# basilevh/occlusions-4d

Hardware: AMD Instinct MI355X
Metric: 4D query-points/sec (encode+decode) at n_points=14336 (higher is better)
Workload: dtype f32; 1 GPU; GREATER inference (BASELINE configs[1]): n_points=14336 video_len=12 num_sample=524288 (-> 534528 grid queries) implicit_batch_size=32768 (decoded in mini-batches of 32256 = 3584 workgroups of 9 queries; every query is decoded, results do not depend on the split), seeded random-init weights; abstract_points=531, outputs_per_query=5, parallelism=single GPU, schedule=sequential, rccl_ranks=1, decode_streams=2, decode_chunk=32256

## Files before the change

### occlusions-4d_amd/csrc/tile.hpp

```cpp
#pragma once
#include "common.hpp"

namespace {

typedef float f32x2 __attribute__((ext_vector_type(2)));
typedef float f32x4 __attribute__((ext_vector_type(4)));
typedef float f32x16 __attribute__((ext_vector_type(16)));
typedef unsigned u32x2 __attribute__((ext_vector_type(2)));
typedef unsigned u32x4 __attribute__((ext_vector_type(4)));

template <typename T>
__device__ __forceinline__ unsigned lds_addr(const T* p) {
  return (unsigned)(uintptr_t)(const __attribute__((address_space(3))) T*)p;
}

template <typename T>
__device__ __forceinline__ void dma_frag(const T* __restrict__ src_frag, unsigned lds_dst, unsigned lane16) {
  unsigned keep;
  asm volatile("s_mov_b32 %0, m0\n\ts_mov_b32 m0, %2\n\ts_nop 0\n\tglobal_load_lds_dwordx4 %1, %3\n\ts_mov_b32 m0, %0"
               : "=&s"(keep) : "v"(lane16), "s"(lds_dst), "s"(src_frag) : "memory");
}
__device__ __forceinline__ void dma_wait() { asm volatile("s_waitcnt vmcnt(0)" ::: "memory"); }

__device__ __forceinline__ f32x4 relu4(f32x4 v) {
  v.x = fmaxf(v.x, 0.f); v.y = fmaxf(v.y, 0.f); v.z = fmaxf(v.z, 0.f); v.w = fmaxf(v.w, 0.f);
  return v;
}

struct Pair { float lo, hi; };
__device__ __forceinline__ Pair swap16(float x, float y) {
  const auto r = __builtin_amdgcn_permlane16_swap(__float_as_uint(x), __float_as_uint(y), false, false);
  return Pair{__uint_as_float(r[0]), __uint_as_float(r[1])};
}
__device__ __forceinline__ Pair swap32(float x, float y) {
  const auto r = __builtin_amdgcn_permlane32_swap(__float_as_uint(x), __float_as_uint(y), false, false);
  return Pair{__uint_as_float(r[0]), __uint_as_float(r[1])};
}

__device__ __forceinline__ void mfma16x2(const f32x4 a0, const f32x4 a1, const f32x4 b0, const f32x4 b1, f32x4& c0, f32x4& c1) {
  c0 = __builtin_amdgcn_mfma_f32_16x16x4f32(a0.x, b0.x, c0, 0, 0, 0);
  c1 = __builtin_amdgcn_mfma_f32_16x16x4f32(a1.x, b1.x, c1, 0, 0, 0);
  c0 = __builtin_amdgcn_mfma_f32_16x16x4f32(a0.y, b0.y, c0, 0, 0, 0);
  c1 = __builtin_amdgcn_mfma_f32_16x16x4f32(a1.y, b1.y, c1, 0, 0, 0);
  c0 = __builtin_amdgcn_mfma_f32_16x16x4f32(a0.z, b0.z, c0, 0, 0, 0);
  c1 = __builtin_amdgcn_mfma_f32_16x16x4f32(a1.z, b1.z, c1, 0, 0, 0);
  c0 = __builtin_amdgcn_mfma_f32_16x16x4f32(a0.w, b0.w, c0, 0, 0, 0);
  c1 = __builtin_amdgcn_mfma_f32_16x16x4f32(a1.w, b1.w, c1, 0, 0, 0);
}
__device__ __forceinline__ void mfma16x2_a(const f32x4 a, const f32x4 b0, const f32x4 b1, f32x4& c0, f32x4& c1) {
  mfma16x2(a, a, b0, b1, c0, c1);
}
__device__ __forceinline__ void mfma16x2_b(const f32x4 a0, const f32x4 a1, const f32x4 b, f32x4& c0, f32x4& c1) {
  mfma16x2(a0, a1, b, b, c0, c1);
}

}
```

### occlusions-4d_amd/csrc/trunk.hip

```cpp
#include "tile.hpp"

namespace {

constexpr int TH = 416;
constexpr int TKG = TH / 16;
constexpr int TNS = TH / 32;
constexpr int FRAG_FLOATS = 256;
constexpr int STAGE_FRAGS = 2 * TKG;
constexpr int STAGE_FLOATS = STAGE_FRAGS * FRAG_FLOATS;
constexpr int TROWS = 128;

struct TrunkArgs {
  const float* x; int64_t ldx;
  float* y; int64_t ldy;
  const float* w0p; const float* b0;
  const float* w1p; const float* b1;
  const float* res; int64_t ldr;
  const float* zconst; const float* ztab; int64_t ldz; const int32_t* zidx; const float* zw; int kz;
  int n;
  int n_stages;
  int relu_in;
  const float* mask; int64_t ldm;
};

__device__ __forceinline__ void dma_stage(const float* __restrict__ src, const float* dst, int wave, int lane) {
#pragma unroll
  for (int i = 0; i < 7; ++i) {
    const int c = wave + 8 * i;
    if (c < STAGE_FRAGS) dma_frag(src + c * FRAG_FLOATS, lds_addr(dst) + (unsigned)c * (FRAG_FLOATS * 4), (unsigned)lane * 16u);
  }
}

__device__ __forceinline__ void dma_part(const float* __restrict__ src, const float* dst, int wave, int lane, int i) {
  const int c = wave + 8 * i;
  if (c < STAGE_FRAGS) dma_frag(src + c * FRAG_FLOATS, lds_addr(dst) + (unsigned)c * (FRAG_FLOATS * 4), (unsigned)lane * 16u);
}

__device__ __forceinline__ void interp_into(const TrunkArgs& a, int rowc, int g, f32x4* out) {
#pragma unroll
  for (int t = 0; t < TKG; ++t) {
    const f32x4 c = *reinterpret_cast<const f32x4*>(a.zconst + 16 * t + 4 * g);
    out[t].x += c.x; out[t].y += c.y; out[t].z += c.z; out[t].w += c.w;
  }
  for (int j = 0; j < a.kz; ++j) {
    const float w = a.zw[(int64_t)rowc * a.kz + j];
    const float* zr = a.ztab + (int64_t)a.zidx[(int64_t)rowc * a.kz + j] * a.ldz + 4 * g;
#pragma unroll
    for (int t = 0; t < TKG; ++t) {
      const f32x4 z = *reinterpret_cast<const f32x4*>(zr + 16 * t);
      out[t].x = fmaf(w, z.x, out[t].x); out[t].y = fmaf(w, z.y, out[t].y);
      out[t].z = fmaf(w, z.z, out[t].z); out[t].w = fmaf(w, z.w, out[t].w);
    }
  }
}

__global__ __launch_bounds__(512, 2) void resblock_kernel(const TrunkArgs a) {
  __shared__ __attribute__((aligned(16))) float bufA[STAGE_FLOATS];
  __shared__ __attribute__((aligned(16))) float bufB[STAGE_FLOATS];
  __shared__ __attribute__((aligned(16))) float s_b0[TH];
  const int tid = threadIdx.x, lane = tid & 63, wave = __builtin_amdgcn_readfirstlane(tid >> 6);
  const int r = lane & 15, g = lane >> 4;
  const int row = blockIdx.x * TROWS + wave * 16 + r;
  const int rowc = min(row, a.n - 1);

  dma_stage(a.w0p, bufA, wave, lane);
  if (tid < TH) s_b0[tid] = a.b0[tid];
  f32x4 xr[TKG], yacc[TKG];
  {
    const float* xp = a.x + (int64_t)rowc * a.ldx + 4 * g;
#pragma unroll
    for (int t = 0; t < TKG; ++t) {
#ifdef OCC4D_TR_NOPRO
      const f32x4 v = {(float)t, (float)g, (float)r, 1.f};
#else
      const f32x4 v = *reinterpret_cast<const f32x4*>(xp + 16 * t);
#endif
      const f32x4 b = *reinterpret_cast<const f32x4*>(a.b1 + 16 * t + 4 * g);
      xr[t] = relu4(v);
      yacc[t].x = v.x + b.x; yacc[t].y = v.y + b.y; yacc[t].z = v.z + b.z; yacc[t].w = v.w + b.w;
    }
  }
  dma_wait();
  __syncthreads();
  const float* const fa = bufA + lane * 4;
  const float* const fb = bufB + lane * 4;

#ifdef OCC4D_TR_STAMP
  unsigned long long tacc[4] = {0, 0, 0, 0};
  unsigned long long tprev = __builtin_amdgcn_s_memtime();
  const unsigned long long tstart = tprev;
#define STAMP(i) { const unsigned long long tn = __builtin_amdgcn_s_memtime(); tacc[i] += tn - tprev; tprev = tn; }
#else
#define STAMP(i)
#endif
  asm volatile("; OCC4D_MARK loop");
#pragma clang loop unroll(disable)
  for (int j = 0; j < TNS; ++j) {
    f32x4 h0 = *reinterpret_cast<const f32x4*>(s_b0 + 32 * j + 4 * g);
    f32x4 h1 = *reinterpret_cast<const f32x4*>(s_b0 + 32 * j + 16 + 4 * g);
    {
      f32x4 wa = *reinterpret_cast<const f32x4*>(fa);
      f32x4 wb = *reinterpret_cast<const f32x4*>(fa + TKG * FRAG_FLOATS);
#pragma unroll
      for (int t = 0; t < TKG; ++t) {
#ifndef OCC4D_TR_NODMA
        if (t >= 2 && t <= 20 && (t - 2) % 3 == 0) dma_part(a.w1p + (int64_t)j * STAGE_FLOATS, bufB, wave, lane, (t - 2) / 3);
#endif
        const f32x4 ca = wa, cb = wb;
        if (t + 1 < TKG) {
          wa = *reinterpret_cast<const f32x4*>(fa + (t + 1) * FRAG_FLOATS);
          wb = *reinterpret_cast<const f32x4*>(fa + (TKG + t + 1) * FRAG_FLOATS);
        }
        __builtin_amdgcn_sched_barrier(0);
        mfma16x2_b(ca, cb, xr[t], h0, h1);
        __builtin_amdgcn_sched_barrier(0);
      }
    }
    h0 = relu4(h0);
    h1 = relu4(h1);
    STAMP(0)
#ifndef OCC4D_TR_NOBAR
    dma_wait();
    __syncthreads();
#endif
    STAMP(1)
    {
      f32x4 wa = *reinterpret_cast<const f32x4*>(fb);
      f32x4 wb = *reinterpret_cast<const f32x4*>(fb + 2 * FRAG_FLOATS);
#pragma unroll
      for (int q = 0; q < TKG; ++q) {
        const int p = q >> 1, tt = q & 1;
#ifndef OCC4D_TR_NODMA
        if (q >= 2 && q <= 20 && (q - 2) % 3 == 0) dma_part(a.w0p + (int64_t)(j + 1) * STAGE_FLOATS, bufA, wave, lane, (q - 2) / 3);
#endif
        const f32x4 ca = wa, cb = wb;
        if (q + 1 < TKG) {
          const int pn = (q + 1) >> 1, tn = (q + 1) & 1;
          wa = *reinterpret_cast<const f32x4*>(fb + (4 * pn + tn) * FRAG_FLOATS);
          wb = *reinterpret_cast<const f32x4*>(fb + (4 * pn + 2 + tn) * FRAG_FLOATS);
        }
        __builtin_amdgcn_sched_barrier(0);
        mfma16x2_b(ca, cb, tt ? h1 : h0, yacc[2 * p], yacc[2 * p + 1]);
        __builtin_amdgcn_sched_barrier(0);
      }
    }
    STAMP(2)
#ifndef OCC4D_TR_NOBAR
    dma_wait();
    __syncthreads();
#endif
    STAMP(3)
  }
  asm volatile("; OCC4D_MARK epilogue");
#ifdef OCC4D_TR_STAMP
  if (lane == 0 && a.zw) {
    unsigned long long* o = (unsigned long long*)a.zw + (size_t)(blockIdx.x * 8 + wave) * 6;
    o[0] = tacc[0]; o[1] = tacc[1]; o[2] = tacc[2]; o[3] = tacc[3]; o[4] = tprev - tstart; o[5] = tstart;
  }
#endif
  if (a.ztab) interp_into(a, rowc, g, yacc);
#ifdef OCC4D_TR_NOEPI
  {
    float tsum = 0.f;
#pragma unroll
    for (int t = 0; t < TKG; ++t) tsum += yacc[t].x + yacc[t].y + yacc[t].z + yacc[t].w;
    if (tsum == 123.456f) a.y[0] = tsum;
    return;
  }
#endif
  if (row < a.n) {
    float* yp = a.y + (int64_t)row * a.ldy + 4 * g;
#pragma unroll
    for (int t = 0; t < TKG; ++t) *reinterpret_cast<f32x4*>(yp + 16 * t) = yacc[t];
  }
}

__device__ __forceinline__ void rowlin_stage(const TrunkArgs& a, int s, const float* __restrict__ frag, const f32x4* xr,
                                             int row, int rowc, int g, const float* next_src, const float* next_dst,
                                             int wave, int lane) {
  const int c0 = 32 * s + 4 * g;
  const f32x4 bz0 = *reinterpret_cast<const f32x4*>(a.b0 + c0);
  const f32x4 bz1 = *reinterpret_cast<const f32x4*>(a.b0 + c0 + 16);
  f32x4 o0 = {0.f, 0.f, 0.f, 0.f}, o1 = {0.f, 0.f, 0.f, 0.f};
  f32x4 r0 = {0.f, 0.f, 0.f, 0.f}, r1 = {0.f, 0.f, 0.f, 0.f};
  if (a.res) {
    r0 = *reinterpret_cast<const f32x4*>(a.res + (int64_t)rowc * a.ldr + c0);
    r1 = *reinterpret_cast<const f32x4*>(a.res + (int64_t)rowc * a.ldr + c0 + 16);
  }
  {
    f32x4 wa = *reinterpret_cast<const f32x4*>(frag);
    f32x4 wb = *reinterpret_cast<const f32x4*>(frag + TKG * FRAG_FLOATS);
#pragma unroll
    for (int t = 0; t < TKG; ++t) {
      if (t >= 2 && t <= 20 && (t - 2) % 3 == 0) dma_part(next_src, next_dst, wave, lane, (t - 2) / 3);
      const f32x4 ca = wa, cb = wb;
      if (t + 1 < TKG) {
        wa = *reinterpret_cast<const f32x4*>(frag + (t + 1) * FRAG_FLOATS);
        wb = *reinterpret_cast<const f32x4*>(frag + (TKG + t + 1) * FRAG_FLOATS);
      }
      __builtin_amdgcn_sched_barrier(0);
      mfma16x2_b(ca, cb, xr[t], o0, o1);
      __builtin_amdgcn_sched_barrier(0);
    }
  }
  o0.x += bz0.x + r0.x; o0.y += bz0.y + r0.y; o0.z += bz0.z + r0.z; o0.w += bz0.w + r0.w;
  o1.x += bz1.x + r1.x; o1.y += bz1.y + r1.y; o1.z += bz1.z + r1.z; o1.w += bz1.w + r1.w;
  if (a.ztab) {
    const f32x4 ca = *reinterpret_cast<const f32x4*>(a.zconst + c0);
    const f32x4 cb = *reinterpret_cast<const f32x4*>(a.zconst + c0 + 16);
    o0.x += ca.x; o0.y += ca.y; o0.z += ca.z; o0.w += ca.w;
    o1.x += cb.x; o1.y += cb.y; o1.z += cb.z; o1.w += cb.w;
    for (int j = 0; j < a.kz; ++j) {
      const float w = a.zw[(int64_t)rowc * a.kz + j];
      const float* zr = a.ztab + (int64_t)a.zidx[(int64_t)rowc * a.kz + j] * a.ldz + c0;
      const f32x4 za = *reinterpret_cast<const f32x4*>(zr);
      const f32x4 zb = *reinterpret_cast<const f32x4*>(zr + 16);
      o0.x = fmaf(w, za.x, o0.x); o0.y = fmaf(w, za.y, o0.y); o0.z = fmaf(w, za.z, o0.z); o0.w = fmaf(w, za.w, o0.w);
      o1.x = fmaf(w, zb.x, o1.x); o1.y = fmaf(w, zb.y, o1.y); o1.z = fmaf(w, zb.z, o1.z); o1.w = fmaf(w, zb.w, o1.w);
    }
  }
  if (a.mask) {
    const f32x4 m0 = *reinterpret_cast<const f32x4*>(a.mask + (int64_t)rowc * a.ldm + c0);
    const f32x4 m1 = *reinterpret_cast<const f32x4*>(a.mask + (int64_t)rowc * a.ldm + c0 + 16);
    o0.x = m0.x > 0.f ? o0.x : 0.f; o0.y = m0.y > 0.f ? o0.y : 0.f; o0.z = m0.z > 0.f ? o0.z : 0.f; o0.w = m0.w > 0.f ? o0.w : 0.f;
    o1.x = m1.x > 0.f ? o1.x : 0.f; o1.y = m1.y > 0.f ? o1.y : 0.f; o1.z = m1.z > 0.f ? o1.z : 0.f; o1.w = m1.w > 0.f ? o1.w : 0.f;
  }
  if (row < a.n) {
    float* yp = a.y + (int64_t)row * a.ldy + c0;
    *reinterpret_cast<f32x4*>(yp) = o0;
    *reinterpret_cast<f32x4*>(yp + 16) = o1;
  }
}

__global__ __launch_bounds__(512, 2) void rowlin_kernel(const TrunkArgs a) {
  __shared__ __attribute__((aligned(16))) float bufA[STAGE_FLOATS];
  __shared__ __attribute__((aligned(16))) float bufB[STAGE_FLOATS];
  const int tid = threadIdx.x, lane = tid & 63, wave = __builtin_amdgcn_readfirstlane(tid >> 6);
  const int r = lane & 15, g = lane >> 4;
  const int row = blockIdx.x * TROWS + wave * 16 + r;
  const int rowc = min(row, a.n - 1);
  dma_stage(a.w0p, bufA, wave, lane);
  f32x4 xr[TKG];
  {
    const float* xp = a.x + (int64_t)rowc * a.ldx + 4 * g;
#pragma unroll
    for (int t = 0; t < TKG; ++t) {
      const f32x4 v = *reinterpret_cast<const f32x4*>(xp + 16 * t);
      xr[t] = a.relu_in ? relu4(v) : v;
    }
  }
  dma_wait();
  __syncthreads();
#pragma clang loop unroll(disable)
  for (int s = 0; s < a.n_stages; s += 2) {
    rowlin_stage(a, s, bufA + lane * 4, xr, row, rowc, g, a.w0p + (int64_t)(s + 1) * STAGE_FLOATS, bufB, wave, lane);
    dma_wait();
    __syncthreads();
    if (s + 1 < a.n_stages)
      rowlin_stage(a, s + 1, bufB + lane * 4, xr, row, rowc, g, a.w0p + (int64_t)(s + 2) * STAGE_FLOATS, bufA, wave, lane);
    dma_wait();
    __syncthreads();
  }
}

int rowlin_launch(const char* who, const float* x, int64_t ldx, float* y, int64_t ldy, const float* w_packed, const float* b,
                  int n_out, int relu_in, const float* res, int64_t ldr, const float* zconst, const float* ztab, int64_t ldz,
                  const int32_t* zidx, const float* zw, int kz, bool masked, const float* mask, int64_t ldm, int n,
                  void* stream) {
  if (n == 0) return OCC4D_OK;
  TrunkArgs a{x, ldx, y, ldy, w_packed, b, nullptr, nullptr, res, ldr, zconst, ztab, ldz, zidx, zw, kz, n,
              n_out / 32, relu_in, mask, ldm};
  if (int rc = occ4d::check_rowlin_args(a, who, TH, 32, n_out, masked)) return rc;
  rowlin_kernel<<<occ4d::cdiv(n, TROWS), 512, 0, (hipStream_t)stream>>>(a);
  return occ4d::check_launch(who);
}

}

extern "C" int occ4d_trunk_width(void) { return TH; }
extern "C" int64_t occ4d_trunk_packed_floats(int n_out) { return (int64_t)(n_out / 32 + 1) * STAGE_FLOATS; }

extern "C" int occ4d_resblock_f32(const float* x, int64_t ldx, float* y, int64_t ldy, const float* w0_packed,
                                  const float* b0, const float* w1_packed, const float* b1, const float* zconst,
                                  const float* ztab, int64_t ldz, const int32_t* zidx, const float* zw, int kz, int n,
                                  void* stream) {
  TrunkArgs a{x, ldx, y, ldy, w0_packed, b0, w1_packed, b1, nullptr, 0, zconst, ztab, ldz, zidx, zw, kz, n, TNS, 1, nullptr, 0};
  if (n == 0) return OCC4D_OK;
  if (int rc = occ4d::check_trunk_args(a, "occ4d_resblock_f32", TH)) return rc;
  OCC4D_REQUIRE(w1_packed && b1 && ((uintptr_t)w1_packed % 16) == 0 && ((uintptr_t)b1 % 16) == 0 && ldy >= TH,
                "occ4d_resblock_f32: second layer weights / bias missing or misaligned");
  resblock_kernel<<<occ4d::cdiv(n, TROWS), 512, 0, (hipStream_t)stream>>>(a);
  return occ4d::check_launch("occ4d_resblock_f32");
}

extern "C" int occ4d_rowlin_f32(const float* x, int64_t ldx, float* y, int64_t ldy, const float* w_packed,
                                const float* b, int n_out, int relu_in, const float* res, int64_t ldr,
                                const float* zconst, const float* ztab, int64_t ldz, const int32_t* zidx,
                                const float* zw, int kz, int n, void* stream) {
  return rowlin_launch("occ4d_rowlin_f32", x, ldx, y, ldy, w_packed, b, n_out, relu_in, res, ldr, zconst, ztab, ldz, zidx, zw,
                       kz, false, nullptr, 0, n, stream);
}

extern "C" int occ4d_rowlin_masked_f32(const float* x, int64_t ldx, float* y, int64_t ldy, const float* w_packed,
                                       const float* b, int n_out, int relu_in, const float* res, int64_t ldr,
                                       const float* mask, int64_t ldm, int n, void* stream) {
  return rowlin_launch("occ4d_rowlin_masked_f32", x, ldx, y, ldy, w_packed, b, n_out, relu_in, res, ldr, nullptr, nullptr, 0,
                       nullptr, nullptr, 0, true, mask, ldm, n, stream);
}
```

### profiles/ablate_trunk.py

```python
import ctypes as C
import os
import subprocess
import sys

import torch

ROOT = os.path.dirname(os.path.dirname(os.path.abspath(__file__)))
sys.path.insert(0, ROOT)
import occlusions4d_amd as pk

CSRC = os.path.join(ROOT, 'occlusions-4d_amd', 'csrc')
VARIANTS = {
    'base': [],
    'nodma': ['-DOCC4D_TR_NODMA'],
    'nobar': ['-DOCC4D_TR_NOBAR'],
    'nodma-nobar': ['-DOCC4D_TR_NODMA', '-DOCC4D_TR_NOBAR'],
    'nopro': ['-DOCC4D_TR_NOPRO'],
    'noepi': ['-DOCC4D_TR_NOEPI'],
    'nopro-noepi': ['-DOCC4D_TR_NOPRO', '-DOCC4D_TR_NOEPI'],
    'bare-loop': ['-DOCC4D_TR_NOPRO', '-DOCC4D_TR_NOEPI', '-DOCC4D_TR_NODMA', '-DOCC4D_TR_NOBAR'],
}


def main():
    n, H = 32256, 416
    x = torch.randn(n, H, device='cuda')
    w0 = torch.randn(H, H, device='cuda') * 0.05
    w1 = torch.randn(H, H, device='cuda') * 0.05
    b = torch.randn(H, device='cuda')
    y = torch.empty(n, H, device='cuda')
    p0, p1 = pk.ops.pack_trunk_rows(w0), pk.ops.pack_trunk_cols(w1)
    names = sys.argv[1:] or list(VARIANTS)
    extra = os.environ.get('OCC4D_ABLATE_EXTRA', '').split()
    for name in names:
        out = '/tmp/trunk_%s.so' % name
        subprocess.run(['hipcc', '--offload-arch=gfx950', '-O3', '-std=c++17', '-ffp-contract=off', '-fPIC', '-shared',
                        '-I' + os.path.join(ROOT, 'include'), '-I' + CSRC] + VARIANTS[name] + extra +
                       [os.path.join(CSRC, 'trunk.hip'), os.path.join(CSRC, 'error.hip'), '-o', out], check=True)
        lib = C.CDLL(out)
        fn = lib.occ4d_resblock_f32
        fn.restype = C.c_int
        fn.argtypes = pk._lib.SIGNATURES['occ4d_resblock_f32'][1]
        run = lambda: fn(x.data_ptr(), H, y.data_ptr(), H, p0.data_ptr(), b.data_ptr(), p1.data_ptr(), b.data_ptr(),
                         None, None, 0, None, None, 0, n, None)
        assert run() == 0
        torch.cuda.synchronize()
        e0, e1 = torch.cuda.Event(enable_timing=True), torch.cuda.Event(enable_timing=True)
        e0.record()
        for _ in range(20):
            run()
        e1.record()
        torch.cuda.synchronize()
        us = e0.elapsed_time(e1) / 20 * 1e3
        print('%-14s %8.1f us  %6.1f TFLOP/s  %.3f of peak' % (name, us, 4.0 * n * H * H / us / 1e6, 4.0 * n * H * H / us / 1e6 / 157.3),
              flush=True)


if __name__ == '__main__':
    main()
```

Measured before the change: 4.579 million query-points/s.

## Overlap trunk prologue loads and output stores with MFMA weight stages

The resblock and rowlin kernels now issue their input-row and bias loads as asynchronous inline-asm global loads. Each row tile is waited on with a per-tile vmcnt just before its first MFMA use, so the prologue latency overlaps the first GEMM stage. The resblock output stores are spread across the final stage's MFMA groups, and rowlin defers each stage's store into the next stage. The point is to hide global-memory latency at kernel start and end. The price is fragile hand-computed vmcnt counts that depend on the DMA schedule, plus heavy template recursion.

```diff
diff --git a/occlusions-4d_amd/csrc/tile.hpp b/occlusions-4d_amd/csrc/tile.hpp
--- a/occlusions-4d_amd/csrc/tile.hpp
+++ b/occlusions-4d_amd/csrc/tile.hpp
@@ -21,6 +21,23 @@
                : "=&s"(keep) : "v"(lane16), "s"(lds_dst), "s"(src_frag) : "memory");
 }
 __device__ __forceinline__ void dma_wait() { asm volatile("s_waitcnt vmcnt(0)" ::: "memory"); }
+
+template <int BYTE_OFF>
+__device__ __forceinline__ void load4_async(f32x4& dst, const float* base) {
+  asm volatile("global_load_dwordx4 %0, %1, off offset:%2" : "=v"(dst) : "v"(base), "n"(BYTE_OFF) : "memory");
+}
+__device__ __forceinline__ void load1_async(float& dst, const float* p) {
+  asm volatile("global_load_dword %0, %1, off" : "=v"(dst) : "v"(p) : "memory");
+}
+template <int N>
+__device__ __forceinline__ void vm_wait(f32x4& a) { asm volatile("s_waitcnt vmcnt(%1)" : "+v"(a) : "n"(N) : "memory"); }
+template <int N>
+__device__ __forceinline__ void vm_wait(f32x4& a, f32x4& b) {
+  asm volatile("s_waitcnt vmcnt(%2)" : "+v"(a), "+v"(b) : "n"(N) : "memory");
+}
+template <int N>
+__device__ __forceinline__ void vm_wait(float& a) { asm volatile("s_waitcnt vmcnt(%1)" : "+v"(a) : "n"(N) : "memory"); }
+__device__ __forceinline__ void lds_barrier() { asm volatile("s_waitcnt lgkmcnt(0)\n\ts_barrier" ::: "memory"); }
 
 __device__ __forceinline__ f32x4 relu4(f32x4 v) {
   v.x = fmaxf(v.x, 0.f); v.y = fmaxf(v.y, 0.f); v.z = fmaxf(v.z, 0.f); v.w = fmaxf(v.w, 0.f);
diff --git a/occlusions-4d_amd/csrc/trunk.hip b/occlusions-4d_amd/csrc/trunk.hip
--- a/occlusions-4d_amd/csrc/trunk.hip
+++ b/occlusions-4d_amd/csrc/trunk.hip
@@ -54,34 +54,144 @@
   }
 }
 
+constexpr int ROW_LOADS =
+#ifdef OCC4D_TR_NOPRO
+    0;
+#else
+    TKG;
+#endif
+__host__ __device__ constexpr int tile_wait_count(int t) {
+#ifdef OCC4D_TR_NODMA
+  return ROW_LOADS ? TKG - 1 - t : 0;
+#else
+  return (ROW_LOADS ? TKG - 1 - t : 0) + (t <= 2 ? 0 : ((t - 3) / 3 + 1 < 6 ? (t - 3) / 3 + 1 : 6));
+#endif
+}
+
+template <int T = 0>
+__device__ __forceinline__ void issue_row_tiles(const float* xp, f32x4* v, int g, int r) {
+  if constexpr (T < TKG) {
+#ifdef OCC4D_TR_NOPRO
+    v[T] = f32x4{(float)T, (float)g, (float)r, 1.f};
+#else
+    load4_async<64 * T>(v[T], xp);
+#endif
+    issue_row_tiles<T + 1>(xp, v, g, r);
+  }
+}
+template <int T>
+__device__ __forceinline__ f32x4 bias_tile(const f32x4& cb0, const f32x4& cb1, int baddr) {
+  const f32x4 c = T < 16 ? cb0 : cb1;
+  const int ad = baddr + 4 * (T & 15);
+  f32x4 b;
+  b.x = __int_as_float(__builtin_amdgcn_ds_bpermute(ad, __float_as_int(c.x)));
+  b.y = __int_as_float(__builtin_amdgcn_ds_bpermute(ad, __float_as_int(c.y)));
+  b.z = __int_as_float(__builtin_amdgcn_ds_bpermute(ad, __float_as_int(c.z)));
+  b.w = __int_as_float(__builtin_amdgcn_ds_bpermute(ad, __float_as_int(c.w)));
+  return b;
+}
+
+struct BiasTiles { f32x4 cb0, cb1; int baddr; };
+template <bool FIRST, int T = 0>
+__device__ __forceinline__ void resblock_groups_a(const TrunkArgs& a, int j, const float* fa, const float* bufB, f32x4* xr,
+                                                  f32x4* yacc, f32x4& wa, f32x4& wb, f32x4& h0, f32x4& h1, int wave, int lane,
+                                                  const BiasTiles& bt) {
+  if constexpr (T < TKG) {
+    if constexpr (FIRST) {
+      const f32x4 b = bias_tile<T>(bt.cb0, bt.cb1, bt.baddr);
+      vm_wait<tile_wait_count(T)>(xr[T]);
+      const f32x4 v = xr[T];
+      yacc[T].x = v.x + b.x; yacc[T].y = v.y + b.y; yacc[T].z = v.z + b.z; yacc[T].w = v.w + b.w;
+      xr[T] = relu4(v);
+      asm volatile("" : "+v"(yacc[T]));
+    }
+#ifndef OCC4D_TR_NODMA
+    if constexpr (T >= 2 && T <= 20 && (T - 2) % 3 == 0) dma_part(a.w1p + (int64_t)j * STAGE_FLOATS, bufB, wave, lane, (T - 2) / 3);
+#endif
+    const f32x4 ca = wa, cb = wb;
+    if constexpr (T + 1 < TKG) {
+      wa = *reinterpret_cast<const f32x4*>(fa + (T + 1) * FRAG_FLOATS);
+      wb = *reinterpret_cast<const f32x4*>(fa + (TKG + T + 1) * FRAG_FLOATS);
+    }
+    __builtin_amdgcn_sched_barrier(0);
+    mfma16x2_b(ca, cb, xr[T], h0, h1);
+    __builtin_amdgcn_sched_barrier(0);
+    resblock_groups_a<FIRST, T + 1>(a, j, fa, bufB, xr, yacc, wa, wb, h0, h1, wave, lane, bt);
+  }
+}
+template <bool FIRST>
+__device__ __forceinline__ void resblock_stage_a(const TrunkArgs& a, int j, const float* fa, const float* bufB, const float* s_b0,
+                                                 f32x4* xr, f32x4* yacc, f32x4& h0, f32x4& h1, int g, int wave, int lane,
+                                                 const BiasTiles& bt) {
+  h0 = *reinterpret_cast<const f32x4*>(s_b0 + 32 * j + 4 * g);
+  h1 = *reinterpret_cast<const f32x4*>(s_b0 + 32 * j + 16 + 4 * g);
+  f32x4 wa = *reinterpret_cast<const f32x4*>(fa);
+  f32x4 wb = *reinterpret_cast<const f32x4*>(fa + TKG * FRAG_FLOATS);
+  resblock_groups_a<FIRST>(a, j, fa, bufB, xr, yacc, wa, wb, h0, h1, wave, lane, bt);
+  h0 = relu4(h0);
+  h1 = relu4(h1);
+}
+
+template <bool LAST, int Q = 0>
+__device__ __forceinline__ void resblock_groups_b(const TrunkArgs& a, int j, const float* fb, const float* bufA, f32x4* yacc,
+                                                  f32x4& wa, f32x4& wb, const f32x4& h0, const f32x4& h1, float* yp, int wave,
+                                                  int lane) {
+  if constexpr (Q < TKG) {
+    constexpr int p = Q >> 1, tt = Q & 1;
+    if constexpr (LAST) {
+#ifndef OCC4D_TR_NOEPI
+      if constexpr (Q >= 3 && tt == 1) {
+        if (yp) {
+          *reinterpret_cast<f32x4*>(yp + 16 * (Q - 3)) = yacc[Q - 3];
+          *reinterpret_cast<f32x4*>(yp + 16 * (Q - 2)) = yacc[Q - 2];
+        }
+      }
+#endif
+    } else {
+#ifndef OCC4D_TR_NODMA
+      if constexpr (Q >= 2 && Q <= 20 && (Q - 2) % 3 == 0) dma_part(a.w0p + (int64_t)(j + 1) * STAGE_FLOATS, bufA, wave, lane, (Q - 2) / 3);
+#endif
+    }
+    const f32x4 ca = wa, cb = wb;
+    if constexpr (Q + 1 < TKG) {
+      constexpr int pn = (Q + 1) >> 1, tn = (Q + 1) & 1;
+      wa = *reinterpret_cast<const f32x4*>(fb + (4 * pn + tn) * FRAG_FLOATS);
+      wb = *reinterpret_cast<const f32x4*>(fb + (4 * pn + 2 + tn) * FRAG_FLOATS);
+    }
+    __builtin_amdgcn_sched_barrier(0);
+    mfma16x2_b(ca, cb, tt ? h1 : h0, yacc[2 * p], yacc[2 * p + 1]);
+    __builtin_amdgcn_sched_barrier(0);
+    resblock_groups_b<LAST, Q + 1>(a, j, fb, bufA, yacc, wa, wb, h0, h1, yp, wave, lane);
+  }
+}
+template <bool LAST>
+__device__ __forceinline__ void resblock_stage_b(const TrunkArgs& a, int j, const float* fb, const float* bufA, f32x4* yacc,
+                                                 const f32x4& h0, const f32x4& h1, float* yp, int wave, int lane) {
+  f32x4 wa = *reinterpret_cast<const f32x4*>(fb);
+  f32x4 wb = *reinterpret_cast<const f32x4*>(fb + 2 * FRAG_FLOATS);
+  resblock_groups_b<LAST>(a, j, fb, bufA, yacc, wa, wb, h0, h1, yp, wave, lane);
+}
+
 __global__ __launch_bounds__(512, 2) void resblock_kernel(const TrunkArgs a) {
   __shared__ __attribute__((aligned(16))) float bufA[STAGE_FLOATS];
   __shared__ __attribute__((aligned(16))) float bufB[STAGE_FLOATS];
   __shared__ __attribute__((aligned(16))) float s_b0[TH];
   const int tid = threadIdx.x, lane = tid & 63, wave = __builtin_amdgcn_readfirstlane(tid >> 6);
   const int r = lane & 15, g = lane >> 4;
-  const int row = blockIdx.x * TROWS + wave * 16 + r;
-  const int rowc = min(row, a.n - 1);
 
   dma_stage(a.w0p, bufA, wave, lane);
-  if (tid < TH) s_b0[tid] = a.b0[tid];
   f32x4 xr[TKG], yacc[TKG];
-  {
-    const float* xp = a.x + (int64_t)rowc * a.ldx + 4 * g;
-#pragma unroll
-    for (int t = 0; t < TKG; ++t) {
-#ifdef OCC4D_TR_NOPRO
-      const f32x4 v = {(float)t, (float)g, (float)r, 1.f};
-#else
-      const f32x4 v = *reinterpret_cast<const f32x4*>(xp + 16 * t);
-#endif
-      const f32x4 b = *reinterpret_cast<const f32x4*>(a.b1 + 16 * t + 4 * g);
-      xr[t] = relu4(v);
-      yacc[t].x = v.x + b.x; yacc[t].y = v.y + b.y; yacc[t].z = v.z + b.z; yacc[t].w = v.w + b.w;
-    }
-  }
-  dma_wait();
-  __syncthreads();
+  float vb0;
+  BiasTiles bt;
+  bt.baddr = 64 * g;
+  load1_async(vb0, a.b0 + min(tid, TH - 1));
+  load4_async<0>(bt.cb0, a.b1 + 16 * r + 4 * g);
+  load4_async<0>(bt.cb1, a.b1 + 16 * min(16 + r, TKG - 1) + 4 * g);
+  issue_row_tiles(a.x + (int64_t)min((int)blockIdx.x * TROWS + wave * 16 + r, a.n - 1) * a.ldx + 4 * g, xr, g, r);
+  vm_wait<ROW_LOADS>(vb0);
+  vm_wait<ROW_LOADS>(bt.cb0, bt.cb1);
+  if (tid < TH) s_b0[tid] = vb0;
+  lds_barrier();
   const float* const fa = bufA + lane * 4;
   const float* const fb = bufB + lane * 4;
 
@@ -93,64 +203,44 @@
 #else
 #define STAMP(i)
 #endif
+#ifndef OCC4D_TR_NOBAR
+#define STAGE_SYNC() { dma_wait(); __syncthreads(); }
+#else
+#define STAGE_SYNC()
+#endif
   asm volatile("; OCC4D_MARK loop");
+  f32x4 h0, h1;
+  resblock_stage_a<true>(a, 0, fa, bufB, s_b0, xr, yacc, h0, h1, g, wave, lane, bt);
+  STAMP(0)
+  STAGE_SYNC()
+  STAMP(1)
+  resblock_stage_b<false>(a, 0, fb, bufA, yacc, h0, h1, nullptr, wave, lane);
+  STAMP(2)
+  STAGE_SYNC()
+  STAMP(3)
 #pragma clang loop unroll(disable)
-  for (int j = 0; j < TNS; ++j) {
-    f32x4 h0 = *reinterpret_cast<const f32x4*>(s_b0 + 32 * j + 4 * g);
-    f32x4 h1 = *reinterpret_cast<const f32x4*>(s_b0 + 32 * j + 16 + 4 * g);
-    {
-      f32x4 wa = *reinterpret_cast<const f32x4*>(fa);
-      f32x4 wb = *reinterpret_cast<const f32x4*>(fa + TKG * FRAG_FLOATS);
-#pragma unroll
-      for (int t = 0; t < TKG; ++t) {
-#ifndef OCC4D_TR_NODMA
-        if (t >= 2 && t <= 20 && (t - 2) % 3 == 0) dma_part(a.w1p + (int64_t)j * STAGE_FLOATS, bufB, wave, lane, (t - 2) / 3);
-#endif
-        const f32x4 ca = wa, cb = wb;
-        if (t + 1 < TKG) {
-          wa = *reinterpret_cast<const f32x4*>(fa + (t + 1) * FRAG_FLOATS);
-          wb = *reinterpret_cast<const f32x4*>(fa + (TKG + t + 1) * FRAG_FLOATS);
-        }
-        __builtin_amdgcn_sched_barrier(0);
-        mfma16x2_b(ca, cb, xr[t], h0, h1);
-        __builtin_amdgcn_sched_barrier(0);
-      }
-    }
-    h0 = relu4(h0);
-    h1 = relu4(h1);
+  for (int j = 1; j < TNS - 1; ++j) {
+    resblock_stage_a<false>(a, j, fa, bufB, s_b0, xr, yacc, h0, h1, g, wave, lane, bt);
     STAMP(0)
-#ifndef OCC4D_TR_NOBAR
-    dma_wait();
-    __syncthreads();
-#endif
+    STAGE_SYNC()
     STAMP(1)
-    {
-      f32x4 wa = *reinterpret_cast<const f32x4*>(fb);
-      f32x4 wb = *reinterpret_cast<const f32x4*>(fb + 2 * FRAG_FLOATS);
-#pragma unroll
-      for (int q = 0; q < TKG; ++q) {
-        const int p = q >> 1, tt = q & 1;
-#ifndef OCC4D_TR_NODMA
-        if (q >= 2 && q <= 20 && (q - 2) % 3 == 0) dma_part(a.w0p + (int64_t)(j + 1) * STAGE_FLOATS, bufA, wave, lane, (q - 2) / 3);
-#endif
-        const f32x4 ca = wa, cb = wb;
-        if (q + 1 < TKG) {
-          const int pn = (q + 1) >> 1, tn = (q + 1) & 1;
-          wa = *reinterpret_cast<const f32x4*>(fb + (4 * pn + tn) * FRAG_FLOATS);
-          wb = *reinterpret_cast<const f32x4*>(fb + (4 * pn + 2 + tn) * FRAG_FLOATS);
-        }
-        __builtin_amdgcn_sched_barrier(0);
-        mfma16x2_b(ca, cb, tt ? h1 : h0, yacc[2 * p], yacc[2 * p + 1]);
-        __builtin_amdgcn_sched_barrier(0);
-      }
-    }
+    resblock_stage_b<false>(a, j, fb, bufA, yacc, h0, h1, nullptr, wave, lane);
     STAMP(2)
-#ifndef OCC4D_TR_NOBAR
-    dma_wait();
-    __syncthreads();
-#endif
+    STAGE_SYNC()
     STAMP(3)
   }
+  resblock_stage_a<false>(a, TNS - 1, fa, bufB, s_b0, xr, yacc, h0, h1, g, wave, lane, bt);
+  STAMP(0)
+  STAGE_SYNC()
+  STAMP(1)
+  int tid_out = tid;
+  asm volatile("" : "+v"(tid_out));
+  const int row = blockIdx.x * TROWS + (tid_out >> 6) * 16 + (tid_out & 15);
+  const int rowc = min(row, a.n - 1);
+  float* const yrow = a.y + (int64_t)row * a.ldy + 4 * ((tid_out & 63) >> 4);
+  const bool streamed = !a.ztab;
+  resblock_stage_b<true>(a, TNS - 1, fb, bufA, yacc, h0, h1, (streamed && row < a.n) ? yrow : nullptr, wave, lane);
+  STAMP(2)
   asm volatile("; OCC4D_MARK epilogue");
 #ifdef OCC4D_TR_STAMP
   if (lane == 0 && a.zw) {
@@ -169,39 +259,76 @@
   }
 #endif
   if (row < a.n) {
-    float* yp = a.y + (int64_t)row * a.ldy + 4 * g;
+    if (streamed) {
+      *reinterpret_cast<f32x4*>(yrow + 16 * (TKG - 2)) = yacc[TKG - 2];
+      *reinterpret_cast<f32x4*>(yrow + 16 * (TKG - 1)) = yacc[TKG - 1];
+    } else {
 #pragma unroll
-    for (int t = 0; t < TKG; ++t) *reinterpret_cast<f32x4*>(yp + 16 * t) = yacc[t];
-  }
-}
-
-__device__ __forceinline__ void rowlin_stage(const TrunkArgs& a, int s, const float* __restrict__ frag, const f32x4* xr,
+      for (int t = 0; t < TKG; ++t) *reinterpret_cast<f32x4*>(yrow + 16 * t) = yacc[t];
+    }
+  }
+#undef STAGE_SYNC
+}
+
+template <bool FIRST, int T = 0>
+__device__ __forceinline__ void rowlin_groups(const TrunkArgs& a, const float* __restrict__ frag, f32x4* xr, f32x4& wa, f32x4& wb,
+                                              f32x4& o0, f32x4& o1, const float* next_src, const float* next_dst, int wave,
+                                              int lane) {
+  if constexpr (T < TKG) {
+    if constexpr (FIRST) {
+      vm_wait<tile_wait_count(T)>(xr[T]);
+      if (a.relu_in) xr[T] = relu4(xr[T]);
+    }
+#ifndef OCC4D_TR_NODMA
+    if constexpr (T >= 2 && T <= 20 && (T - 2) % 3 == 0) dma_part(next_src, next_dst, wave, lane, (T - 2) / 3);
+#endif
+    const f32x4 ca = wa, cb = wb;
+    if constexpr (T + 1 < TKG) {
+      wa = *reinterpret_cast<const f32x4*>(frag + (T + 1) * FRAG_FLOATS);
+      wb = *reinterpret_cast<const f32x4*>(frag + (TKG + T + 1) * FRAG_FLOATS);
+    }
+    __builtin_amdgcn_sched_barrier(0);
+    mfma16x2_b(ca, cb, xr[T], o0, o1);
+    __builtin_amdgcn_sched_barrier(0);
+    rowlin_groups<FIRST, T + 1>(a, frag, xr, wa, wb, o0, o1, next_src, next_dst, wave, lane);
+  }
+}
+
+__device__ __forceinline__ void rowlin_store(const TrunkArgs& a, int s, int row, int g, const f32x4& o0, const f32x4& o1) {
+#ifdef OCC4D_TR_NOST
+  if (o0.x + o1.x != 123.456f) return;
+#endif
+  if (row < a.n) {
+    float* yp = a.y + (int64_t)row * a.ldy + 32 * s + 4 * g;
+    *reinterpret_cast<f32x4*>(yp) = o0;
+    *reinterpret_cast<f32x4*>(yp + 16) = o1;
+  }
+}
+
+template <bool FIRST>
+__device__ __forceinline__ void rowlin_stage(const TrunkArgs& a, int s, const float* __restrict__ frag, f32x4* xr,
                                              int row, int rowc, int g, const float* next_src, const float* next_dst,
-                                             int wave, int lane) {
+                                             int wave, int lane, f32x4& p0, f32x4& p1) {
   const int c0 = 32 * s + 4 * g;
-  const f32x4 bz0 = *reinterpret_cast<const f32x4*>(a.b0 + c0);
-  const f32x4 bz1 = *reinterpret_cast<const f32x4*>(a.b0 + c0 + 16);
+  if constexpr (!FIRST) rowlin_store(a, s - 1, row, g, p0, p1);
+  f32x4 bz0, bz1;
+  f32x4 r0 = {0.f, 0.f, 0.f, 0.f}, r1 = {0.f, 0.f, 0.f, 0.f};
+  bz0 = *reinterpret_cast<const f32x4*>(a.b0 + c0);
+  bz1 = *reinterpret_cast<const f32x4*>(a.b0 + c0 + 16);
   f32x4 o0 = {0.f, 0.f, 0.f, 0.f}, o1 = {0.f, 0.f, 0.f, 0.f};
-  f32x4 r0 = {0.f, 0.f, 0.f, 0.f}, r1 = {0.f, 0.f, 0.f, 0.f};
   if (a.res) {
     r0 = *reinterpret_cast<const f32x4*>(a.res + (int64_t)rowc * a.ldr + c0);
     r1 = *reinterpret_cast<const f32x4*>(a.res + (int64_t)rowc * a.ldr + c0 + 16);
   }
+  if constexpr (FIRST) {
+    issue_row_tiles(a.x + (int64_t)rowc * a.ldx + 4 * g, xr, g, lane & 15);
+    asm volatile("s_waitcnt vmcnt(%0)" :: "n"(ROW_LOADS) : "memory");
+    lds_barrier();
+  }
   {
     f32x4 wa = *reinterpret_cast<const f32x4*>(frag);
     f32x4 wb = *reinterpret_cast<const f32x4*>(frag + TKG * FRAG_FLOATS);
-#pragma unroll
-    for (int t = 0; t < TKG; ++t) {
-      if (t >= 2 && t <= 20 && (t - 2) % 3 == 0) dma_part(next_src, next_dst, wave, lane, (t - 2) / 3);
-      const f32x4 ca = wa, cb = wb;
-      if (t + 1 < TKG) {
-        wa = *reinterpret_cast<const f32x4*>(frag + (t + 1) * FRAG_FLOATS);
-        wb = *reinterpret_cast<const f32x4*>(frag + (TKG + t + 1) * FRAG_FLOATS);
-      }
-      __builtin_amdgcn_sched_barrier(0);
-      mfma16x2_b(ca, cb, xr[t], o0, o1);
-      __builtin_amdgcn_sched_barrier(0);
-    }
+    rowlin_groups<FIRST>(a, frag, xr, wa, wb, o0, o1, next_src, next_dst, wave, lane);
   }
   o0.x += bz0.x + r0.x; o0.y += bz0.y + r0.y; o0.z += bz0.z + r0.z; o0.w += bz0.w + r0.w;
   o1.x += bz1.x + r1.x; o1.y += bz1.y + r1.y; o1.z += bz1.z + r1.z; o1.w += bz1.w + r1.w;
@@ -225,11 +352,8 @@
     o0.x = m0.x > 0.f ? o0.x : 0.f; o0.y = m0.y > 0.f ? o0.y : 0.f; o0.z = m0.z > 0.f ? o0.z : 0.f; o0.w = m0.w > 0.f ? o0.w : 0.f;
     o1.x = m1.x > 0.f ? o1.x : 0.f; o1.y = m1.y > 0.f ? o1.y : 0.f; o1.z = m1.z > 0.f ? o1.z : 0.f; o1.w = m1.w > 0.f ? o1.w : 0.f;
   }
-  if (row < a.n) {
-    float* yp = a.y + (int64_t)row * a.ldy + c0;
-    *reinterpret_cast<f32x4*>(yp) = o0;
-    *reinterpret_cast<f32x4*>(yp + 16) = o1;
-  }
+  p0 = o0;
+  p1 = o1;
 }
 
 __global__ __launch_bounds__(512, 2) void rowlin_kernel(const TrunkArgs a) {
@@ -240,27 +364,21 @@
   const int row = blockIdx.x * TROWS + wave * 16 + r;
   const int rowc = min(row, a.n - 1);
   dma_stage(a.w0p, bufA, wave, lane);
-  f32x4 xr[TKG];
-  {
-    const float* xp = a.x + (int64_t)rowc * a.ldx + 4 * g;
-#pragma unroll
-    for (int t = 0; t < TKG; ++t) {
-      const f32x4 v = *reinterpret_cast<const f32x4*>(xp + 16 * t);
-      xr[t] = a.relu_in ? relu4(v) : v;
-    }
-  }
+  f32x4 xr[TKG], p0, p1;
+  rowlin_stage<true>(a, 0, bufA + lane * 4, xr, row, rowc, g, a.w0p + (int64_t)STAGE_FLOATS, bufB, wave, lane, p0, p1);
   dma_wait();
   __syncthreads();
 #pragma clang loop unroll(disable)
-  for (int s = 0; s < a.n_stages; s += 2) {
-    rowlin_stage(a, s, bufA + lane * 4, xr, row, rowc, g, a.w0p + (int64_t)(s + 1) * STAGE_FLOATS, bufB, wave, lane);
+  for (int s = 1; s < a.n_stages; s += 2) {
+    rowlin_stage<false>(a, s, bufB + lane * 4, xr, row, rowc, g, a.w0p + (int64_t)(s + 1) * STAGE_FLOATS, bufA, wave, lane, p0, p1);
     dma_wait();
     __syncthreads();
     if (s + 1 < a.n_stages)
-      rowlin_stage(a, s + 1, bufB + lane * 4, xr, row, rowc, g, a.w0p + (int64_t)(s + 2) * STAGE_FLOATS, bufA, wave, lane);
+      rowlin_stage<false>(a, s + 1, bufA + lane * 4, xr, row, rowc, g, a.w0p + (int64_t)(s + 2) * STAGE_FLOATS, bufB, wave, lane, p0, p1);
     dma_wait();
     __syncthreads();
   }
+  rowlin_store(a, a.n_stages - 1, row, g, p0, p1);
 }
 
 int rowlin_launch(const char* who, const float* x, int64_t ldx, float* y, int64_t ldy, const float* w_packed, const float* b,
diff --git a/profiles/ablate_trunk.py b/profiles/ablate_trunk.py
--- a/profiles/ablate_trunk.py
+++ b/profiles/ablate_trunk.py
@@ -9,7 +9,8 @@
 sys.path.insert(0, ROOT)
 import occlusions4d_amd as pk
 
-CSRC = os.path.join(ROOT, 'occlusions-4d_amd', 'csrc')
+CSRC = os.environ.get('OCC4D_ABLATE_CSRC', os.path.join(ROOT, 'occlusions-4d_amd', 'csrc'))
+LIBDIR = os.environ.get('OCC4D_ABLATE_LIBDIR', '/tmp')
 VARIANTS = {
     'base': [],
     'nodma': ['-DOCC4D_TR_NODMA'],
@@ -19,7 +20,35 @@
     'noepi': ['-DOCC4D_TR_NOEPI'],
     'nopro-noepi': ['-DOCC4D_TR_NOPRO', '-DOCC4D_TR_NOEPI'],
     'bare-loop': ['-DOCC4D_TR_NOPRO', '-DOCC4D_TR_NOEPI', '-DOCC4D_TR_NODMA', '-DOCC4D_TR_NOBAR'],
+    'nost': ['-DOCC4D_TR_NOST'],
+    'nopro-nost': ['-DOCC4D_TR_NOPRO', '-DOCC4D_TR_NOST'],
 }
+ROWLIN_VARIANTS = ('base', 'nopro', 'nost', 'nopro-nost')
+
+
+def compile_variant(name, out):
+    extra = os.environ.get('OCC4D_ABLATE_EXTRA', '').split()
+    subprocess.run(['hipcc', '--offload-arch=gfx950', '-O3', '-std=c++17', '-ffp-contract=off', '-fno-honor-nans', '-fPIC',
+                    '-shared', '-I' + os.path.join(ROOT, 'include'), '-I' + CSRC] + VARIANTS[name] + extra +
+                   [os.path.join(CSRC, 'trunk.hip'), os.path.join(CSRC, 'error.hip'), '-o', out], check=True)
+
+
+def timed(run, reps=40, batches=5):
+    assert run() == 0
+    for _ in range(reps):
+        run()
+    torch.cuda.synchronize()
+    got = []
+    for _ in range(batches):
+        e0, e1 = torch.cuda.Event(enable_timing=True), torch.cuda.Event(enable_timing=True)
+        e0.record()
+        for _ in range(reps):
+            run()
+        e1.record()
+        torch.cuda.synchronize()
+        got.append(e0.elapsed_time(e1) / reps * 1e3)
+    got.sort()
+    return got[len(got) // 2], got[0], got[-1]
 
 
 def main():
@@ -27,33 +56,41 @@
     x = torch.randn(n, H, device='cuda')
     w0 = torch.randn(H, H, device='cuda') * 0.05
     w1 = torch.randn(H, H, device='cuda') * 0.05
-    b = torch.randn(H, device='cuda')
+    w2 = torch.randn(2 * H, H, device='cuda') * 0.05
+    b = torch.randn(2 * H, device='cuda')
     y = torch.empty(n, H, device='cuda')
-    p0, p1 = pk.ops.pack_trunk_rows(w0), pk.ops.pack_trunk_cols(w1)
+    y2 = torch.empty(n, 2 * H, device='cuda')
+    acc = torch.randn(n, H, device='cuda')
+    p0, p1, p2 = pk.ops.pack_trunk_rows(w0), pk.ops.pack_trunk_cols(w1), pk.ops.pack_trunk_rows(w2)
     names = sys.argv[1:] or list(VARIANTS)
-    extra = os.environ.get('OCC4D_ABLATE_EXTRA', '').split()
+    for _ in range(300):
+        pk.ops.resblock(x, p0, b[:H], p1, b[:H], out=y)
+    torch.cuda.synchronize()
     for name in names:
-        out = '/tmp/trunk_%s.so' % name
-        subprocess.run(['hipcc', '--offload-arch=gfx950', '-O3', '-std=c++17', '-ffp-contract=off', '-fPIC', '-shared',
-                        '-I' + os.path.join(ROOT, 'include'), '-I' + CSRC] + VARIANTS[name] + extra +
-                       [os.path.join(CSRC, 'trunk.hip'), os.path.join(CSRC, 'error.hip'), '-o', out], check=True)
+        out = os.path.join(LIBDIR, 'trunk_%s.so' % name)
+        if not os.path.exists(out):
+            compile_variant(name, out)
         lib = C.CDLL(out)
-        fn = lib.occ4d_resblock_f32
-        fn.restype = C.c_int
-        fn.argtypes = pk._lib.SIGNATURES['occ4d_resblock_f32'][1]
-        run = lambda: fn(x.data_ptr(), H, y.data_ptr(), H, p0.data_ptr(), b.data_ptr(), p1.data_ptr(), b.data_ptr(),
-                         None, None, 0, None, None, 0, n, None)
-        assert run() == 0
-        torch.cuda.synchronize()
-        e0, e1 = torch.cuda.Event(enable_timing=True), torch.cuda.Event(enable_timing=True)
-        e0.record()
-        for _ in range(20):
-            run()
-        e1.record()
-        torch.cuda.synchronize()
-        us = e0.elapsed_time(e1) / 20 * 1e3
-        print('%-14s %8.1f us  %6.1f TFLOP/s  %.3f of peak' % (name, us, 4.0 * n * H * H / us / 1e6, 4.0 * n * H * H / us / 1e6 / 157.3),
-              flush=True)
+        res = lib.occ4d_resblock_f32
+        res.restype = C.c_int
+        res.argtypes = pk._lib.SIGNATURES['occ4d_resblock_f32'][1]
+        lin = lib.occ4d_rowlin_f32
+        lin.restype = C.c_int
+        lin.argtypes = pk._lib.SIGNATURES['occ4d_rowlin_f32'][1]
+        launches = [('resblock', 4.0 * n * H * H, lambda: res(
+            x.data_ptr(), H, y.data_ptr(), H, p0.data_ptr(), b.data_ptr(), p1.data_ptr(), b.data_ptr(),
+            None, None, 0, None, None, 0, n, None))]
+        if name in ROWLIN_VARIANTS:
+            launches += [('rowlin 416->832', 4.0 * n * H * H, lambda: lin(
+                x.data_ptr(), H, y2.data_ptr(), 2 * H, p2.data_ptr(), b.data_ptr(), 2 * H, 0, None, 0,
+                None, None, 0, None, None, 0, n, None)),
+                ('rowlin 416->416 +res', 2.0 * n * H * H, lambda: lin(
+                    x.data_ptr(), H, acc.data_ptr(), H, p0.data_ptr(), b.data_ptr(), H, 0, acc.data_ptr(), H,
+                    None, None, 0, None, None, 0, n, None))]
+        for what, flops, run in launches:
+            us, lo, hi = timed(run)
+            print('%-12s %-22s %8.1f us [%.1f, %.1f]  %6.1f TFLOP/s  %.3f of peak' % (
+                name, what, us, lo, hi, flops / us / 1e6, flops / us / 1e6 / 157.3), flush=True)
 
 
 if __name__ == '__main__':
```

After: 4.619 million query-points/s, median of 6. Within noise of the previous version (+0.9%).
